# nagadomi/nunif

Hardware: AMD Instinct MI355X
Metric: input MPix/s, waifu2x swin_unet 2x tiled render (tile 256) of 1080p frames (higher is better)
Workload: dtype f16; 1 GPU; waifu2x swin_unet 2x (art scale2x geometry), tile_size=256, 1080p frame, random-init weights; tile_size=256, tile_batch=45, tiles_per_frame=45, concurrent_streams=2, parallelism=frame-sharded x1

## Files before the change

nunif_amd/csrc/swin_qkv_attn_r.hip:

```cpp
#include <algorithm>
#include <cstdlib>

#include "swin_kernels.h"

namespace nunif {


constexpr float kRegionR = 100.0f;

struct QkvAttnRArgs {
    const f16 *x;
    f16 *att;
    const f16 *wres;
    const float *bqkv;
    const float *btab32;
    int B, H, W, shift, n_windows;
    int rev;
};

__device__ __forceinline__ f16x4 mul4_to_f16(const f32x4 &o, float inv) {
    return (f16x4){(f16)__builtin_fmaf(o[0], inv, 0.0f), (f16)__builtin_fmaf(o[1], inv, 0.0f), (f16)__builtin_fmaf(o[2], inv, 0.0f),
                   (f16)__builtin_fmaf(o[3], inv, 0.0f)};
}
__device__ __forceinline__ f16x4 lone_to_f16x4(float e, float zf) {
    return (f16x4){(f16)e, (f16)zf, (f16)0.f, (f16)0.f};
}

constexpr int kBiasStride = 52;


__device__ __host__ inline int win_token(int mt, int r16) { return mt < 2 ? 16 * mt + r16 : ((r16 & 3) == 0 ? 32 + (r16 >> 2) : 35); }

template <int C, int HD, int HPP, int WAVES = 8, bool WM = false>
__global__ void __launch_bounds__(WAVES * 64)
qkv_attn_r_kernel(QkvAttnRArgs a) {
    constexpr int kWavesR = WAVES;
    constexpr int NTHR = WAVES * 64;
    constexpr int KS = C / 32;
    constexpr int HEADS = C / HD;
    constexpr int NTH = HD / 16;
    constexpr int FPH = 3 * NTH * KS;
    constexpr int PASSES = HEADS / HPP;
    static_assert(HEADS == 6 && HEADS % HPP == 0, "swin_unet uses 6 heads at every level");
    extern __shared__ __attribute__((aligned(16))) unsigned char smem_r[];
    f16x8 *wl = reinterpret_cast<f16x8 *>(smem_r);
    float *bt32 = reinterpret_cast<float *>(wl + HPP * FPH * 64);
    float *bl = bt32 + HPP * kQkvBiasFloatsPerHead;

    const int tid = threadIdx.x;
    const int lane = tid & 63;
    const int wave = __builtin_amdgcn_readfirstlane(tid >> 6);
    const int r16 = lane & 15;
    const int grp = lane >> 4;
    const int nwx = a.W / 6, nwy = a.H / 6;
    const f16x4 zero4 = {(f16)0.f, (f16)0.f, (f16)0.f, (f16)0.f};
    float zf = 0.f;
    asm("" : "+s"(zf));

    for (int i = tid; i < 3 * C; i += NTHR) bl[i] = a.bqkv[i];
    const f16x8 ones8 = {(f16)1.f, (f16)1.f, (f16)1.f, (f16)1.f, (f16)1.f, (f16)1.f, (f16)1.f, (f16)1.f};

    int tokc[3];
#pragma unroll
    for (int mt = 0; mt < 3; ++mt) tokc[mt] = win_token(mt, r16);
    unsigned wm_off[3];
#pragma unroll
    for (int mt = 0; mt < 3; ++mt) wm_off[mt] = (unsigned)((tokc[mt] * HD + 4 * grp) * 2);
    const bool store2 = (r16 & 3) == 0;
    const int st_delta = (NTH == 2 ? pair_run_channel(grp) : 4 * grp) * 2 - 16 * grp;
    f16x4 rk0 = zero4, rq0 = zero4;
    if (a.shift > 0 && grp == 2) { rk0[0] = (f16)1.f; rq0[0] = (f16)kRegionR; }

    const int n_wg = gridDim.x / PASSES;
    const int wstride = kWavesR * n_wg;
    const bool spread = a.n_windows < 8 * wstride;
    const int w0 = spread ? wave * n_wg + (int)(blockIdx.x / PASSES) : (int)(blockIdx.x / PASSES) * kWavesR + wave;
    const int pass = blockIdx.x % PASSES;
    {
        const f16x8 *src = reinterpret_cast<const f16x8 *>(a.wres) + (long)pass * HPP * FPH * 64;
        for (int i = tid; i < HPP * FPH * 64; i += NTHR) wl[i] = src[i];
        const f32x4 *bsrc = reinterpret_cast<const f32x4 *>(a.btab32 + (long)pass * HPP * kQkvBiasFloatsPerHead);
        for (int i = tid; i < HPP * kQkvBiasFloatsPerHead / 4; i += NTHR) reinterpret_cast<f32x4 *>(bt32)[i] = bsrc[i];
    }
    __syncthreads();

    int cx = w0 % nwx, cy = (w0 / nwx) % nwy, cb = w0 / (nwx * nwy);
    const int dx = wstride % nwx, dy = (wstride / nwx) % nwy, db = wstride / (nwx * nwy);
    const long img_bytes = (long)a.H * a.W * C * 2;

    auto load_x = [&](int wb, int wy, int wx, bool special, f16x8 (&xf)[3][KS], unsigned (&vo)[3]) {
        const int y0 = wy * 6 + a.shift, x0 = wx * 6 + a.shift;
        const char *xb = reinterpret_cast<const char *>(a.x) + (long)wb * img_bytes;
        if (special) {
#pragma unroll
            for (int mt = 0; mt < 3; ++mt) {
                const int tk = win_token(mt, r16), iy = tk / 6, ix = tk - 6 * iy;
                int yy = y0 + iy, xx = x0 + ix;
                if (yy >= a.H) yy -= a.H;
                if (xx >= a.W) xx -= a.W;
                vo[mt] = (unsigned)(((yy * a.W + xx) * C + 8 * grp) * 2);
            }
        } else {
            const unsigned org = (unsigned)((y0 * a.W + x0) * C * 2);
            int rl = r16;
            asm("" : "+v"(rl));
#pragma unroll
            for (int mt = 0; mt < 3; ++mt) {
                const int tk = win_token(mt, rl), iy = (tk * 43) >> 8, ix = tk - 6 * iy;
                vo[mt] = org + (unsigned)(((iy * a.W + ix) * C + 8 * grp) * 2);
            }
        }
#pragma unroll
        for (int mt = 0; mt < 3; ++mt) {
#pragma unroll
            for (int ks = 0; ks < KS; ++ks) xf[mt][ks] = *reinterpret_cast<const f16x8 *>(xb + vo[mt] + 64 * ks);
        }
    };
    auto decode = [&](int &wb, int &wy, int &wx, bool &special) {
        wb = a.rev ? a.B - 1 - cb : cb;
        wy = a.rev ? nwy - 1 - cy : cy;
        wx = a.rev ? nwx - 1 - cx : cx;
        special = a.shift > 0 && (wy == nwy - 1 || wx == nwx - 1);
    };
    auto advance = [&]() {
        cx += dx;
        if (cx >= nwx) { cx -= nwx; ++cy; }
        cy += dy;
        if (cy >= nwy) { cy -= nwy; ++cb; }
        cb += db;
    };

    auto qkv_bias = [&](int hl, int head, int part, int nt) -> f32x4 {
        const int ch0 = part * C + head * HD + nt * 16;
        if (part == 2) { const float bv = bl[ch0 + r16]; return (f32x4){bv, bv, bv, bv}; }
        return *reinterpret_cast<const f32x4 *>(bl + ch0 + 4 * grp);
    };
    auto bias_frag = [&](int hl, int qt, int kt) -> f32x4 {
        return *reinterpret_cast<const f32x4 *>(bt32 + (hl * 36 + tokc[qt]) * kBiasStride + 4 * grp + 16 * kt);
    };
    f16x8 xf[3][KS];
    unsigned vo[3];
    int wb, wy, wx;
    bool special;
    f16x8 wnx = wl[lane];
    auto run_windows = [&]() {
    int wi = w0;
    decode(wb, wy, wx, special);
    auto step = [&]() { advance(); wi += wstride; decode(wb, wy, wx, special); };
    if (wi < a.n_windows) load_x(wb, wy, wx, special, xf, vo);
#pragma unroll 1
    while (wi < a.n_windows) {
        const int wq = (wb * nwy + wy) * nwx + wx;
        char *ab = reinterpret_cast<char *>(a.att) + (WM ? (long)wq * (HEADS * 36 * HD * 2) : (long)wb * img_bytes);
        const unsigned wm_base = (unsigned)__builtin_amdgcn_readfirstlane((unsigned)wq * (unsigned)(HEADS * 36 * HD * 2));

        constexpr bool kEarlyX = C == 96 && WM;
        auto run_heads = [&]() {
        const bool sp_now = special;
        f16x4 rkr[3], rqr[3];
        if (special) {
            const bool last_y = wy == nwy - 1, last_x = wx == nwx - 1;
#pragma unroll
            for (int mt = 0; mt < 3; ++mt) {
                const int tk = win_token(mt, r16), iy = tk / 6, ix = tk - 6 * iy;
                const int reg = ((last_y && iy >= 3) ? 2 : 0) + ((last_x && ix >= 3) ? 1 : 0);
#pragma unroll
                for (int j = 0; j < 4; ++j) {
                    const bool on = grp == 2 && reg == j;
                    rkr[mt][j] = (f16)(on ? 1.f : 0.f);
                    rqr[mt][j] = (f16)(on ? kRegionR : 0.f);
                }
            }
        } else {
#pragma unroll
            for (int mt = 0; mt < 3; ++mt) { rkr[mt] = rk0; rqr[mt] = rq0; }
        }
        constexpr int kHeadUnroll = C == 96 ? HPP : 1;
#pragma unroll kHeadUnroll
        for (int hl = 0; hl < HPP; ++hl) {
            const int head = pass * HPP + hl;
            const f16x8 *wh = wl + (hl * FPH) * 64 + lane;
            constexpr bool kPrefetchW = C == 96;
            f16x4 qt4[NTH][3], kt4[NTH][3], vt4[NTH][3];
            f16x8 wq2[2];
            wq2[0] = kPrefetchW ? wnx : wh[0];
            f32x4 bnx = qkv_bias(hl, head, 0, 0);
#pragma unroll
            for (int part = 0; part < 3; ++part) {
#pragma unroll
                for (int nt = 0; nt < NTH; ++nt) {
                    const int fidx = (part * NTH + nt) * KS;
                    f32x4 acc[3];
                    bnx = qkv_bias(hl, head, part, nt);
#pragma unroll
                    for (int mt = 0; mt < 3; ++mt) acc[mt] = bnx;
#pragma unroll
                    for (int ks = 0; ks < KS; ++ks) {
                        const int f = fidx + ks;
                        if constexpr (kPrefetchW)
                            wq2[(f + 1) & 1] = (f + 1 < FPH) ? wh[(f + 1) * 64] : (hl + 1 < HPP ? wh[FPH * 64] : wl[lane]);
                        else wq2[f & 1] = wh[f * 64];
                        const f16x8 w = wq2[f & 1];
#pragma unroll
                        for (int mt = 0; mt < 3; ++mt)
                            acc[mt] = part == 2 ? MFMA_16x16x32(xf[mt][ks], w, acc[mt]) : MFMA_16x16x32(w, xf[mt][ks], acc[mt]);
                    }
#pragma unroll
                    for (int mt = 0; mt < 3; ++mt) {
                        const f16x4 v = {(f16)acc[mt][0], (f16)acc[mt][1], (f16)acc[mt][2], (f16)acc[mt][3]};
                        if (part == 0) qt4[nt][mt] = v; else if (part == 1) kt4[nt][mt] = v; else vt4[nt][mt] = v;
                    }
                }
            }
            if constexpr (kPrefetchW) wnx = wq2[FPH & 1];
            if constexpr (kEarlyX) {
                if (hl == HPP - 1) {
                    step();
                    if (wi < a.n_windows) load_x(wb, wy, wx, special, xf, vo);
                }
            }

#pragma unroll
            for (int qt = 0; qt < 3; ++qt) {
                f32x4 s[3];
                {
                    f32x4 sb[3];
#pragma unroll
                    for (int kt = 0; kt < 3; ++kt) sb[kt] = bias_frag(hl, qt, kt);
#pragma unroll
                    for (int kt = 0; kt < 3; ++kt) {
                        f32x4 acc = sb[kt];
                        if constexpr (HD == 16) {
                            acc = MFMA_16x16x32(cat8(kt4[0][kt], rkr[kt]), cat8(qt4[0][qt], rqr[qt]), acc);
                        } else {
                            acc = MFMA_16x16x32(cat8(kt4[0][kt], kt4[1][kt]), cat8(qt4[0][qt], qt4[1][qt]), acc);
                            if (sp_now) acc = MFMA_16x16x32(cat8(rkr[kt], zero4), cat8(rqr[qt], zero4), acc);
                        }
                        s[kt] = acc;
                    }
                }
                float mx = fmaxf(fmaxf(fmaxf(fmaxf(s[0][0], s[0][1]), s[0][2]), fmaxf(fmaxf(s[0][3], s[1][0]), s[1][1])),
                                 fmaxf(fmaxf(s[1][2], s[1][3]), s[2][0]));
                mx = row_group_max(mx);
                f16x4 pf[3];
#pragma unroll
                for (int kt = 0; kt < 2; ++kt) {
                    const float p0 = __builtin_amdgcn_exp2f(s[kt][0] - mx), p1 = __builtin_amdgcn_exp2f(s[kt][1] - mx);
                    const float p2 = __builtin_amdgcn_exp2f(s[kt][2] - mx), p3 = __builtin_amdgcn_exp2f(s[kt][3] - mx);
                    pf[kt] = (f16x4){(f16)p0, (f16)p1, (f16)p2, (f16)p3};
                }
                pf[2] = lone_to_f16x4(__builtin_amdgcn_exp2f(s[2][0] - mx), zf);
                const f16x8 psum = cat8(pf[0] + pf[1], pf[2]);
                const f32x4 z4 = {0.f, 0.f, 0.f, 0.f};
                const f32x4 sm = MFMA_16x16x32(ones8, psum, z4);
                const float inv = __builtin_amdgcn_rcpf(sm[0]);
                const bool store = qt < 2 || store2;
                f16x4 ov[NTH];
#pragma unroll
                for (int dt = 0; dt < NTH; ++dt) {
                    f32x4 o = MFMA_16x16x32(cat8(vt4[dt][0], vt4[dt][1]), cat8(pf[0], pf[1]), z4);
                    o = MFMA_16x16x32(cat8(zero4, vt4[dt][2]), psum, o);
                    ov[dt] = mul4_to_f16(o, inv);
                }
                if constexpr (NTH == 2) {
                    const f16x8 run = pair_to_run(ov[0], ov[1]);
                    if (store) *reinterpret_cast<f16x8 *>(ab + (vo[qt] + (unsigned)st_delta) + head * (HD * 2)) = run;
                } else if constexpr (WM) {
                    unsigned long hb = reinterpret_cast<unsigned long>(a.att) + (wm_base + (unsigned)(head * (36 * HD * 2)));
                    asm("" : "+s"(hb));
                    typedef __attribute__((address_space(1))) char gchar;
                    typedef __attribute__((address_space(1))) f16x4 gf16x4;
                    unsigned lo = wm_off[qt];
                    asm("" : "+v"(lo));
                    if (store) *reinterpret_cast<gf16x4 *>(reinterpret_cast<gchar *>(hb) + lo) = ov[0];
                } else {
                    if (store) *reinterpret_cast<f16x4 *>(ab + (vo[qt] + (unsigned)st_delta) + head * (HD * 2)) = ov[0];
                }
            }
            if constexpr (kHeadUnroll > 1) __builtin_amdgcn_sched_barrier(0);
        }
        };
        run_heads();

        if constexpr (!kEarlyX) {
            step();
            if (wi < a.n_windows) load_x(wb, wy, wx, special, xf, vo);
        }
    }
    };
    run_windows();
}

int qkv_attn_r_frags(int C) { return 3 * (C / 16) * (C / 32); }

template <int C, int HD, int HPP, int WAVES = 8, bool WM = false>
static int launch_r(const QkvAttnRArgs &a, int grid, hipStream_t s) {
    constexpr size_t smem = (size_t)HPP * 3 * (HD / 16) * (C / 32) * 1024 + HPP * kQkvBiasFloatsPerHead * 4 + (size_t)3 * C * 4;
    static bool configured = false;
    if (!configured) {
        NUNIF_HIP_CHECK(hipFuncSetAttribute((const void *)qkv_attn_r_kernel<C, HD, HPP, WAVES, WM>,
                                            hipFuncAttributeMaxDynamicSharedMemorySize, (int)smem));
        configured = true;
    }
    qkv_attn_r_kernel<C, HD, HPP, WAVES, WM><<<grid, WAVES * 64, smem, s>>>(a);
    return NUNIF_HIP_OK;
}

int launch_qkv_attn_r(const f16 *x, f16 *att, const f16 *wres, const float *bqkv, const float *btab32,
                      int B, int H, int W, int C, int heads, int shift, hipStream_t s, int rev, int window_major) {
    NUNIF_REQUIRE(H % 6 == 0 && W % 6 == 0, "qkv_attn: %dx%d not a multiple of the 6x6 window", H, W);
    NUNIF_REQUIRE(heads == 6 && (C == 96 || C == 192), "qkv_attn: C=%d heads=%d unsupported", C, heads);
    if (H <= 6) shift = 0;
    QkvAttnRArgs a;
    a.x = x; a.att = att; a.wres = wres; a.bqkv = bqkv; a.btab32 = btab32;
    a.B = B; a.H = H; a.W = W; a.shift = shift;
    a.n_windows = B * (H / 6) * (W / 6);
    a.rev = rev;
    NUNIF_REQUIRE(!window_major || C == 96, "qkv_attn: the window-major att map exists for C = 96 only");
    NUNIF_REQUIRE(!window_major || (long)a.n_windows * (6 * 36 * 16 * 2) < (1L << 32),
                  "qkv_attn: the window-major att map of %d windows does not fit 32-bit byte offsets", a.n_windows);
    const double tok = (double)B * H * W;
    const int kWavesR = C == 96 ? 16 : 8;
    const int wgs = (a.n_windows + kWavesR - 1) / kWavesR;
    int grid = wgs < 256 ? wgs : 256;
    if (C == 192) grid = std::max(2, grid & ~1);
    int rc;
    if (C == 96) {
        ProfScope ps("qkv_attn_r_kernel<96,16>", s, 2.0 * tok * C * 3.0 * C + 4.0 * tok * 36.0 * C, tok * C * 4.0);
        rc = window_major ? launch_r<96, 16, 6, 16, true>(a, grid, s) : launch_r<96, 16, 6, 16, false>(a, grid, s);
    } else {
        ProfScope ps("qkv_attn_r_kernel<192,32>", s, 2.0 * tok * C * 3.0 * C + 4.0 * tok * 36.0 * C, tok * C * 4.0);
        rc = launch_r<192, 32, 3>(a, grid, s);
    }
    if (rc) return rc;
    NUNIF_LAUNCH_CHECK();
    return NUNIF_HIP_OK;
}

}
```

Before: 320.9 MPix/s.

## Pair consecutive windows to share the padded third token tile in C=192 attention

For the C=192 level, each wave now processes two windows back to back. The mostly-padding third M-tile (tokens 32-35) of both windows is packed into one MFMA tile, with the second window's rows carried in the unused lanes. The second window's q/k/v fragments for that tile go through a per-wave LDS stash, so the next window only runs two M-tiles in its QKV projection. This cuts wasted MFMA work on padding rows, but adds LDS, wavefront fences, extra address logic and more register pressure.

```diff
diff --git a/nunif_amd/csrc/swin_qkv_attn_r.hip b/nunif_amd/csrc/swin_qkv_attn_r.hip
--- a/nunif_amd/csrc/swin_qkv_attn_r.hip
+++ b/nunif_amd/csrc/swin_qkv_attn_r.hip
@@ -1,5 +1,6 @@
 #include <algorithm>
 #include <cstdlib>
+#include <type_traits>
 
 #include "swin_kernels.h"
 
@@ -26,6 +27,7 @@
     return (f16x4){(f16)e, (f16)zf, (f16)0.f, (f16)0.f};
 }
 
+constexpr int kAttnStashBytesPerHead = 768;
 constexpr int kBiasStride = 52;
 
 
@@ -46,10 +48,13 @@
     f16x8 *wl = reinterpret_cast<f16x8 *>(smem_r);
     float *bt32 = reinterpret_cast<float *>(wl + HPP * FPH * 64);
     float *bl = bt32 + HPP * kQkvBiasFloatsPerHead;
+    constexpr bool kPair = C == 192;
+    unsigned char *stash = reinterpret_cast<unsigned char *>(bl + 3 * C);
 
     const int tid = threadIdx.x;
     const int lane = tid & 63;
     const int wave = __builtin_amdgcn_readfirstlane(tid >> 6);
+    stash += wave * (HPP * kAttnStashBytesPerHead);
     const int r16 = lane & 15;
     const int grp = lane >> 4;
     const int nwx = a.W / 6, nwy = a.H / 6;
@@ -88,9 +93,8 @@
     const int dx = wstride % nwx, dy = (wstride / nwx) % nwy, db = wstride / (nwx * nwy);
     const long img_bytes = (long)a.H * a.W * C * 2;
 
-    auto load_x = [&](int wb, int wy, int wx, bool special, f16x8 (&xf)[3][KS], unsigned (&vo)[3]) {
+    auto tile_offsets = [&](int wy, int wx, bool special, unsigned (&vo)[3]) {
         const int y0 = wy * 6 + a.shift, x0 = wx * 6 + a.shift;
-        const char *xb = reinterpret_cast<const char *>(a.x) + (long)wb * img_bytes;
         if (special) {
 #pragma unroll
             for (int mt = 0; mt < 3; ++mt) {
@@ -110,8 +114,21 @@
                 vo[mt] = org + (unsigned)(((iy * a.W + ix) * C + 8 * grp) * 2);
             }
         }
+    };
+    auto load_x = [&](int wb, int wy, int wx, bool special, f16x8 (&xf)[3][KS], unsigned (&vo)[3]) {
+        const char *xb = reinterpret_cast<const char *>(a.x) + (long)wb * img_bytes;
+        tile_offsets(wy, wx, special, vo);
 #pragma unroll
         for (int mt = 0; mt < 3; ++mt) {
+#pragma unroll
+            for (int ks = 0; ks < KS; ++ks) xf[mt][ks] = *reinterpret_cast<const f16x8 *>(xb + vo[mt] + 64 * ks);
+        }
+    };
+    auto load_x01 = [&](int wb, int wy, int wx, bool special, f16x8 (&xf)[3][KS], unsigned (&vo)[3]) {
+        const char *xb = reinterpret_cast<const char *>(a.x) + (long)wb * img_bytes;
+        tile_offsets(wy, wx, special, vo);
+#pragma unroll
+        for (int mt = 0; mt < 2; ++mt) {
 #pragma unroll
             for (int ks = 0; ks < KS; ++ks) xf[mt][ks] = *reinterpret_cast<const f16x8 *>(xb + vo[mt] + 64 * ks);
         }
@@ -121,6 +138,17 @@
         wy = a.rev ? nwy - 1 - cy : cy;
         wx = a.rev ? nwx - 1 - cx : cx;
         special = a.shift > 0 && (wy == nwy - 1 || wx == nwx - 1);
+    };
+    auto load_x_pair = [&](int wb, int wy, int wx, bool special, int bb, int by, int bx, f16x8 (&xf)[3][KS], unsigned (&vo)[3]) {
+        load_x01(wb, wy, wx, special, xf, vo);
+        int yy = by * 6 + a.shift + 5, xx = bx * 6 + a.shift + 2 + (r16 >> 2);
+        if (yy >= a.H) yy -= a.H;
+        if (xx >= a.W) xx -= a.W;
+        const unsigned vb = (unsigned)(((yy * a.W + xx) * C + 8 * grp) * 2);
+        const bool own = (r16 & 3) == 0;
+        const char *p2 = reinterpret_cast<const char *>(a.x) + ((long)(own ? wb : bb) * img_bytes + (own ? vo[2] : vb));
+#pragma unroll
+        for (int ks = 0; ks < KS; ++ks) xf[2][ks] = *reinterpret_cast<const f16x8 *>(p2 + 64 * ks);
     };
     auto advance = [&]() {
         cx += dx;
@@ -147,7 +175,22 @@
     int wi = w0;
     decode(wb, wy, wx, special);
     auto step = [&]() { advance(); wi += wstride; decode(wb, wy, wx, special); };
-    if (wi < a.n_windows) load_x(wb, wy, wx, special, xf, vo);
+    bool paired = false;
+    auto load_trip_a = [&]() {
+        int bb = wb, by = wy, bx = wx;
+        paired = wi + wstride < a.n_windows;
+        if (paired) {
+            const int scx = cx, scy = cy, scb = cb;
+            bool bsp;
+            advance();
+            decode(bb, by, bx, bsp);
+            cx = scx; cy = scy; cb = scb;
+        }
+        load_x_pair(wb, wy, wx, special, bb, by, bx, xf, vo);
+    };
+    if (wi < a.n_windows) {
+        if constexpr (kPair) load_trip_a(); else load_x(wb, wy, wx, special, xf, vo);
+    }
 #pragma unroll 1
     while (wi < a.n_windows) {
         const int wq = (wb * nwy + wy) * nwx + wx;
@@ -155,7 +198,9 @@
         const unsigned wm_base = (unsigned)__builtin_amdgcn_readfirstlane((unsigned)wq * (unsigned)(HEADS * 36 * HD * 2));
 
         constexpr bool kEarlyX = C == 96 && WM;
-        auto run_heads = [&]() {
+        auto run_heads = [&](auto mode_c) {
+        constexpr int MODE = decltype(mode_c)::value;
+        constexpr int MT = MODE == 2 ? 2 : 3;
         const bool sp_now = special;
         f16x4 rkr[3], rqr[3];
         if (special) {
@@ -181,6 +226,8 @@
             const int head = pass * HPP + hl;
             const f16x8 *wh = wl + (hl * FPH) * 64 + lane;
             constexpr bool kPrefetchW = C == 96;
+            unsigned char *sh = stash + hl * kAttnStashBytesPerHead + ((r16 >> 2) * 4 + grp) * 8;
+            unsigned char *shv = stash + hl * kAttnStashBytesPerHead + 512 + lane * 2;
             f16x4 qt4[NTH][3], kt4[NTH][3], vt4[NTH][3];
             f16x8 wq2[2];
             wq2[0] = kPrefetchW ? wnx : wh[0];
@@ -193,7 +240,7 @@
                     f32x4 acc[3];
                     bnx = qkv_bias(hl, head, part, nt);
 #pragma unroll
-                    for (int mt = 0; mt < 3; ++mt) acc[mt] = bnx;
+                    for (int mt = 0; mt < MT; ++mt) acc[mt] = bnx;
 #pragma unroll
                     for (int ks = 0; ks < KS; ++ks) {
                         const int f = fidx + ks;
@@ -202,13 +249,31 @@
                         else wq2[f & 1] = wh[f * 64];
                         const f16x8 w = wq2[f & 1];
 #pragma unroll
-                        for (int mt = 0; mt < 3; ++mt)
+                        for (int mt = 0; mt < MT; ++mt)
                             acc[mt] = part == 2 ? MFMA_16x16x32(xf[mt][ks], w, acc[mt]) : MFMA_16x16x32(w, xf[mt][ks], acc[mt]);
                     }
 #pragma unroll
-                    for (int mt = 0; mt < 3; ++mt) {
+                    for (int mt = 0; mt < MT; ++mt) {
                         const f16x4 v = {(f16)acc[mt][0], (f16)acc[mt][1], (f16)acc[mt][2], (f16)acc[mt][3]};
                         if (part == 0) qt4[nt][mt] = v; else if (part == 1) kt4[nt][mt] = v; else vt4[nt][mt] = v;
+                    }
+                    if constexpr (MODE == 1) {
+                        if (paired) {
+                            if (part < 2) {
+                                if ((r16 & 3) == 1)
+                                    *reinterpret_cast<f16x4 *>(sh + part * 256 + nt * 128) = part == 0 ? qt4[nt][2] : kt4[nt][2];
+                            } else {
+                                *reinterpret_cast<f16 *>(shv + nt * 128) = vt4[nt][2][1];
+                            }
+                        }
+                    }
+                    if constexpr (MODE == 2) {
+                        if (part < 2) {
+                            const f16x4 v = *reinterpret_cast<const f16x4 *>(sh + part * 256 + nt * 128);
+                            if (part == 0) qt4[nt][2] = v; else kt4[nt][2] = v;
+                        } else {
+                            vt4[nt][2] = (f16x4){*reinterpret_cast<const f16 *>(shv + nt * 128), (f16)0.f, (f16)0.f, (f16)0.f};
+                        }
                     }
                 }
             }
@@ -280,11 +345,24 @@
             if constexpr (kHeadUnroll > 1) __builtin_amdgcn_sched_barrier(0);
         }
         };
-        run_heads();
-
-        if constexpr (!kEarlyX) {
+        if constexpr (kPair) {
+            run_heads(std::integral_constant<int, 1>{});
             step();
-            if (wi < a.n_windows) load_x(wb, wy, wx, special, xf, vo);
+            if (paired) {
+                __builtin_amdgcn_fence(__ATOMIC_ACQ_REL, "wavefront");
+                load_x01(wb, wy, wx, special, xf, vo);
+                ab = reinterpret_cast<char *>(a.att) + (long)wb * img_bytes;
+                run_heads(std::integral_constant<int, 2>{});
+                __builtin_amdgcn_fence(__ATOMIC_ACQ_REL, "wavefront");
+                step();
+            }
+            if (wi < a.n_windows) load_trip_a();
+        } else {
+            run_heads(std::integral_constant<int, 0>{});
+            if constexpr (!kEarlyX) {
+                step();
+                if (wi < a.n_windows) load_x(wb, wy, wx, special, xf, vo);
+            }
         }
     }
     };
@@ -295,7 +373,10 @@
 
 template <int C, int HD, int HPP, int WAVES = 8, bool WM = false>
 static int launch_r(const QkvAttnRArgs &a, int grid, hipStream_t s) {
-    constexpr size_t smem = (size_t)HPP * 3 * (HD / 16) * (C / 32) * 1024 + HPP * kQkvBiasFloatsPerHead * 4 + (size_t)3 * C * 4;
+    constexpr size_t smem = (size_t)HPP * 3 * (HD / 16) * (C / 32) * 1024 + HPP * kQkvBiasFloatsPerHead * 4 + (size_t)3 * C * 4 +
+                            (C == 192 ? (size_t)WAVES * HPP * kAttnStashBytesPerHead : 0);
+    static_assert(smem <= 160 * 1024, "qkv_attn_r: over the 160 KiB of LDS of a CU");
+    NUNIF_REQUIRE(smem <= 160 * 1024, "qkv_attn: %zu bytes of LDS, a CU has 160 KiB", smem);
     static bool configured = false;
     if (!configured) {
         NUNIF_HIP_CHECK(hipFuncSetAttribute((const void *)qkv_attn_r_kernel<C, HD, HPP, WAVES, WM>,
```

Result: no change. 322.9 MPix/s (median of 6 runs) (+0.6%).
